# ericbrec/BSpy

Measured on AMD Instinct MI355X. Metric: M evals/sec on 10M-point bicubic (p=3x3) surface, higher is better.
Workload: dtype f64; 1 GPU; BASELINE configs[1]: bicubic surface order 4x4, nCoef 64x64, nDep 3, fp64, clamped uniform knots, Spline.evaluate on 10000000 uniform-random (u,v); points_total=10000000, points_per_gpu=10000000, op=evaluate

## Files before the change

bspy_amd/_native.py:

```python
import ctypes
import os

import numpy as np

_HERE = os.path.dirname(os.path.abspath(__file__))
LIB_PATH = os.environ.get("BSPY_AMD_LIB") or os.path.join(_HERE, "csrc", "libbspy_amd.so")

BSK_F32, BSK_F64 = 0, 1
BSK_HOST, BSK_DEVICE = 0, 1
BSK_OK, BSK_ERR_INVALID, BSK_ERR_DOMAIN, BSK_ERR_HIP, BSK_ERR_NO_DEVICE, BSK_ERR_UNSUPPORTED = range(6)
BSK_MAX_NIND, BSK_MAX_ORDER = 8, 16
BSK_INTEGRAL_MEASURE, BSK_INTEGRAL_NODES = 0, 1

PRODUCT_SYMBOLS = (
    "bsk_version", "bsk_last_error", "bsk_device_count",
    "bsk_spline_create", "bsk_spline_update", "bsk_spline_destroy",
    "bsk_evaluate", "bsk_jacobian", "bsk_normal", "bsk_curvature", "bsk_evaluate_grid", "bsk_tessellate",
    "bsk_domain_status", "bsk_bspline_values", "bsk_last_kernel",
    "bsk_multi_create", "bsk_multi_destroy", "bsk_multi_shard_plan", "bsk_multi_stream", "bsk_multi_evaluate",
    "bsk_multi_jacobian", "bsk_integral",
    "bsk_fit_create", "bsk_fit_destroy", "bsk_fit_info", "bsk_fit_solve_host", "bsk_fit_sweep", "bsk_fit_residual",
    "bsk_fit_last_kernel",
    "bsk_band_create", "bsk_band_destroy", "bsk_band_apply_host", "bsk_band_apply", "bsk_band_last_kernel",
    "bsk_band_absmax", "bsk_band_absmax_host", "bsk_band_apply_fma_host",
    "bsk_product_create", "bsk_product_destroy", "bsk_product_apply_host", "bsk_product_apply", "bsk_product_last_kernel",
    "bsk_scan_create", "bsk_scan_destroy", "bsk_scan_apply_host", "bsk_scan_apply", "bsk_scan_last_kernel",
    "bsk_sum_apply_host", "bsk_sum_apply", "bsk_sum_last_kernel",
    "bsk_roots_extract_host", "bsk_roots_flag_host", "bsk_roots_flag", "bsk_roots_isolate_host", "bsk_roots_isolate", "bsk_roots_last_kernel",
    "bsk_project_seed_host", "bsk_project_seed", "bsk_project_newton_host", "bsk_project_newton", "bsk_project_last_kernel",
    "bsk_contour_flag_host", "bsk_contour_flag", "bsk_contour_march_host", "bsk_contour_march", "bsk_contour_last_kernel",
    "bsk_iso_flag_host", "bsk_iso_flag", "bsk_iso_walk_host", "bsk_iso_walk", "bsk_iso_leaf_host", "bsk_iso_leaf", "bsk_iso_vertex_host",
    "bsk_iso_vertex", "bsk_iso_last_kernel",
    "bsk_mesh_bound_host", "bsk_mesh_bound", "bsk_mesh_count_host", "bsk_mesh_count", "bsk_mesh_emit_host", "bsk_mesh_emit",
    "bsk_mesh_vertex_host", "bsk_mesh_vertex", "bsk_mesh_last_kernel",
    "bsk_rays_boxes_host", "bsk_rays_boxes", "bsk_rays_count_host", "bsk_rays_count", "bsk_rays_emit_host", "bsk_rays_emit",
    "bsk_rays_isolate_host", "bsk_rays_isolate", "bsk_rays_reduce_host", "bsk_rays_reduce", "bsk_rays_last_kernel",
    "bsk_ssx_count_host", "bsk_ssx_count", "bsk_ssx_emit_host", "bsk_ssx_emit", "bsk_ssx_isolate_host", "bsk_ssx_isolate",
    "bsk_ssx_merge_host", "bsk_ssx_merge", "bsk_ssx_last_kernel",
    "bsk_scatter_key_host", "bsk_scatter_key", "bsk_scatter_gram_host", "bsk_scatter_gram", "bsk_scatter_cell_host", "bsk_scatter_cell",
    "bsk_scatter_fold_host", "bsk_scatter_fold", "bsk_scatter_residual_host", "bsk_scatter_residual", "bsk_scatter_solve_host",
    "bsk_scatter_solve_work", "bsk_scatter_solve", "bsk_scatter_reweight_host", "bsk_scatter_reweight", "bsk_scatter_last_kernel",
)
INTERNAL_SYMBOLS = ("bsk_debug_probe", "bsk_debug_stage_times", "bsk_debug_fill_lds", "bsk_debug_scatter_solve")
SYMBOLS = PRODUCT_SYMBOLS + INTERNAL_SYMBOLS
ROOTS2_SYMBOLS = ("bsk_roots2_flag_host", "bsk_roots2_flag", "bsk_roots2_isolate_host", "bsk_roots2_isolate", "bsk_roots2_merge_host",
                  "bsk_roots2_merge", "bsk_roots2_last_kernel")
ROOTS3_SYMBOLS = ("bsk_roots3_flag_host", "bsk_roots3_flag", "bsk_roots3_isolate_host", "bsk_roots3_isolate", "bsk_roots3_merge_host",
                  "bsk_roots3_merge", "bsk_roots3_last_kernel", "bsk_roots3_walk_bound")


class NativeLibraryError(RuntimeError):
    """libbspy_amd.so is missing or failed to load."""


class BskError(RuntimeError):

    def __init__(self, status, message):
        super().__init__(f"libbspy_amd status {status}: {message}")
        self.status = status


class DomainError(Exception):

    def __init__(self, index):
        super().__init__(f"parameter outside domain at flat index {index}")
        self.index = int(index)
# ... 199 lines not shown
    L.bsk_scatter_gram_host.argtypes = gram_s
    L.bsk_scatter_gram.argtypes = gram_s + [_vp]
    L.bsk_scatter_cell_host.argtypes = cell_s
    L.bsk_scatter_cell.argtypes = cell_s + [_vp]
    L.bsk_scatter_fold_host.argtypes = fold_s
    L.bsk_scatter_fold.argtypes = fold_s + [_vp]
    L.bsk_scatter_residual_host.argtypes = residual_s
    L.bsk_scatter_residual.argtypes = residual_s + [_vp]
    L.bsk_scatter_solve_host.argtypes = fold_s + [_i64p]
    reweight_s = [ctypes.c_int, ctypes.c_double, _vp, _vp, _vp, _i64, _vp]
    L.bsk_scatter_solve_work.argtypes = [ctypes.c_int] * 3 + [_i64, _i64, ctypes.c_int, _i64p]
    L.bsk_scatter_solve.argtypes = fold_s + [_vp, _i64, _vp, _vp]
    L.bsk_debug_scatter_solve.argtypes = fold_s + [_vp, _i64, _vp, ctypes.c_int, _vp]
    L.bsk_scatter_reweight_host.argtypes = reweight_s
    L.bsk_scatter_reweight.argtypes = reweight_s + [_vp]
    L.bsk_scatter_last_kernel.argtypes = []
    L.bsk_scatter_last_kernel.restype = ctypes.c_char_p
    L.bsk_last_kernel.argtypes = [_vp]
    L.bsk_last_kernel.restype = ctypes.c_char_p
    L.bsk_debug_probe.argtypes = [_vp, ctypes.c_int, ctypes.c_int, ctypes.c_int, _i64, _vp, _vp, _i64, _vp, _vp]
    L.bsk_debug_stage_times.argtypes = [_vp, ctypes.c_int, ctypes.POINTER(ctypes.c_float), ctypes.POINTER(ctypes.c_char_p),
                                        ctypes.c_int, _ip]
    L.bsk_debug_fill_lds.argtypes = [_vp, ctypes.c_uint32, ctypes.c_int, _i64p, _vp]
    for name in SYMBOLS + ROOTS2_SYMBOLS + ROOTS3_SYMBOLS:
        if name not in ("bsk_version", "bsk_last_error", "bsk_last_kernel", "bsk_fit_last_kernel", "bsk_band_last_kernel",
                        "bsk_product_last_kernel", "bsk_scan_last_kernel", "bsk_sum_last_kernel", "bsk_roots_last_kernel",
                        "bsk_roots2_last_kernel", "bsk_roots3_last_kernel", "bsk_project_last_kernel", "bsk_contour_last_kernel", "bsk_iso_last_kernel", "bsk_mesh_last_kernel", "bsk_rays_last_kernel",
                        "bsk_ssx_last_kernel", "bsk_scatter_last_kernel"):
            getattr(L, name).restype = ctypes.c_int
    _lib = L
    return L


def check(status, first_bad=None):
    if status == BSK_OK:
        return
    if status == BSK_ERR_DOMAIN:
        raise DomainError(first_bad.value if first_bad is not None else -1)
    raise BskError(status, lib().bsk_last_error().decode("utf-8", "replace"))


def device_count():
    n = ctypes.c_int(0)
    st = lib().bsk_device_count(ctypes.byref(n))
    if st != BSK_OK:
        return 0
# ... 17 lines not shown
```

bspy_amd/csrc/bsk_api.hip:

```cpp
#include "bsk_kernels.hpp"
#include "bsk_tile.hpp"
#include "bsk_stream.hpp"
#include "bsk_rowrot.hpp"
#include "bsk_uniform.hpp"
#include "bsk_rec32.hpp"
#include "bsk_host.hpp"

#include <condition_variable>
#include <mutex>
#include <thread>

struct HostPipe;
static void pipe_destroy(HostPipe *p);

static int ceil_log2(int x)
{
    int s = 0;
    while ((1 << s) < x) ++s;
    return s;
}

template <typename T>
static void build_axis_table(const T *knots, int order, int nk, std::vector<T> &tab)
{
// ... 21 lines not shown
static int lut_buckets(int order, int ncoef)
{
    int m = 16;
    while (m < 4 * (ncoef - order + 1) && m < 4096) m <<= 1;
    return m;
}

template <typename T>
static void build_lut(const T *knots, int order, int ncoef, int m, T &scale, int &steps, std::vector<unsigned> &lut)
{
    const double lo = (double)knots[order - 1], hi = (double)knots[ncoef];
    const double w = hi - lo;
    scale = T((double)m / w);
    const double inv = 1.0 / (double)scale;
    int widest = 0;
    for (int b = 0; b < m; ++b) {
        const int l = host_span<T>(knots, order, ncoef, lo + ((double)b - 0.01) * inv);
        const int h = (b == m - 1) ? ncoef : host_span<T>(knots, order, ncoef, lo + ((double)b + 1.01) * inv);
        widest = std::max(widest, h - l);
        lut.push_back((unsigned)l | ((unsigned)h << 16));
    }
    steps = ceil_log2(widest + 1);
}

template <typename T>
static bsk_status upload_tables(bsk_spline s, const void *const *knots, const void *coefs)
{
    Desc<T> &d = desc_of<T>(s);
    TileDesc<T> &td = tile_of<T>(s);
    std::vector<T> tab;
    std::vector<unsigned> lut;
    for (int iv = 0; iv < s->nInd; ++iv) {
        d.off[iv] = (int)tab.size();
        const T *k = static_cast<const T *>(knots[iv]);
        build_axis_table<T>(k, s->order[iv], d.nk[iv], tab);
        d.lo[iv] = k[s->order[iv] - 1];
        d.hi[iv] = k[s->ncoef[iv]];
        td.lut_off[iv] = (int)lut.size();
        const int m_alloc = lut_buckets(s->order[iv], s->ncoef[iv]);
        int m_small = 16;
        while (m_small < s->ncoef[iv] - s->order[iv] + 1) m_small <<= 1;
        std::vector<unsigned> seg;
        int m_use = m_alloc;
        if (m_small < m_alloc) {
            build_lut<T>(k, s->order[iv], s->ncoef[iv], m_small, td.lut_scale[iv], td.lut_steps[iv], seg);
            if (td.lut_steps[iv] <= 1) m_use = m_small;
// ... 2 lines not shown
            seg.clear();
            build_lut<T>(k, s->order[iv], s->ncoef[iv], m_alloc, td.lut_scale[iv], td.lut_steps[iv], seg);
        }
        td.lut_m[iv] = m_use;
        seg.resize((size_t)m_alloc, seg.empty() ? 0u : seg.back());
        lut.insert(lut.end(), seg.begin(), seg.end());
    }
    if ((int)tab.size() != d.tab_len) return fail(BSK_ERR_INVALID, "internal: axis table size changed");
    if ((int)lut.size() != td.lut_len) return fail(BSK_ERR_INVALID, "internal: bucket table size changed");
    HIPCHK(hipSetDevice(s->device));
    if (d.tab_len) HIPCHK(hipMemcpy(s->tab, tab.data(), sizeof(T) * tab.size(), hipMemcpyHostToDevice));
    s->tab_host.assign(reinterpret_cast<const unsigned char *>(tab.data()),
                       reinterpret_cast<const unsigned char *>(tab.data()) + sizeof(T) * tab.size());
    if (td.lut_len) HIPCHK(hipMemcpy(s->lut, lut.data(), sizeof(unsigned) * lut.size(), hipMemcpyHostToDevice));
    if (d.coef_len) HIPCHK(hipMemcpy(s->coef, coefs, sizeof(T) * (size_t)d.coef_len, hipMemcpyHostToDevice));
    if (s->coef_aos) {
        const size_t cells = (size_t)d.coef_len / (size_t)s->nDep;
        std::vector<T> aos((size_t)d.coef_len);
        const T *src = static_cast<const T *>(coefs);
        for (int dep = 0; dep < s->nDep; ++dep)
            for (size_t c = 0; c < cells; ++c) aos[c * s->nDep + dep] = src[(size_t)dep * cells + c];
        HIPCHK(hipMemcpy(s->coef_aos, aos.data(), sizeof(T) * aos.size(), hipMemcpyHostToDevice));
    }
    return BSK_OK;
}

template <typename T>
static bsk_status init_desc(bsk_spline s)
{
    Desc<T> &d = desc_of<T>(s);
    memset(&d, 0, sizeof(d));
    d.nInd = s->nInd;
    d.nDep = s->nDep;
    long long clen = 1;
    long long tlen = 0;
    for (int iv = 0; iv < s->nInd; ++iv) {
        d.order[iv] = s->order[iv];
        d.ncoef[iv] = s->ncoef[iv];
        d.nk[iv] = s->order[iv] + s->ncoef[iv];
        d.steps[iv] = ceil_log2(s->ncoef[iv] - s->order[iv] + 1);
        tlen += (long long)s->order[iv] * d.nk[iv];
        clen *= s->ncoef[iv];
    }
    d.cstride[s->nInd] = 1;
    for (int iv = s->nInd - 1; iv >= 0; --iv) {
        const long long st = (long long)d.cstride[iv + 1] * s->ncoef[iv];
        if (st * std::max(1, s->nDep) > 0x7fffffffLL) return fail(BSK_ERR_UNSUPPORTED, "coefficient table exceeds 2^31 elements");
// ... 105 lines not shown
    s->num_cu = prop.multiProcessorCount > 0 ? prop.multiProcessorCount : 256;
    s->lds_max = std::min<size_t>(160 * 1024, prop.maxSharedMemoryPerMultiProcessor > 0
                                                  ? (size_t)prop.maxSharedMemoryPerMultiProcessor
                                                  : (size_t)64 * 1024);
    HIPCHK_C(hipMalloc(&s->tab, std::max<size_t>(16, s->esize * (size_t)tab_len)));
    HIPCHK_C(hipMalloc(&s->coef, std::max<size_t>(16, s->esize * (size_t)coef_len)));
    {
        const size_t tbytes = s->esize * (size_t)tab_len + s->esize * (size_t)coef_len;
        const int omax = max_order(s);
        const bool fixed = nInd <= 3 && omax <= 6;
        if (fixed && nDep <= 4 && tbytes + 8192 > s->lds_max)
            HIPCHK_C(hipMalloc(&s->coef_aos, std::max<size_t>(16, s->esize * (size_t)coef_len)));
        else if (fixed && nDep <= 4 && nInd == 2 && !s->same_order && omax >= 2) {
            HIPCHK_C(hipMalloc(&s->coef_aos, std::max<size_t>(16, s->esize * (size_t)coef_len)));
            s->aos_small = true;
        }
    }
    HIPCHK_C(hipMalloc((void **)&s->lut, std::max<size_t>(16, sizeof(unsigned) * (size_t)(dtype == BSK_F32 ? s->t32.lut_len : s->t64.lut_len))));
    HIPCHK_C(hipMalloc((void **)&s->bad, 2 * sizeof(unsigned long long)));
    if (const char *v = getenv("BSK_VARIANT")) s->variant = atoi(v);
    HIPCHK_C(hipMemset(s->bad, 0xff, 2 * sizeof(unsigned long long)));
#undef HIPCHK_C
    st = upload_all(s, knots, coefs);
    if (st != BSK_OK) { s->uni_img.release(); cleanup(); return st; }
    *out = s;
    return BSK_OK;
}

extern "C" bsk_status bsk_spline_update(bsk_spline s, const void *const *knots, const void *coefs)
{
    if (!s || !knots || !coefs) return fail(BSK_ERR_INVALID, "NULL argument");
    HIPCHK(hipSetDevice(s->device));
    HIPCHK(hipDeviceSynchronize());
    return upload_all(s, knots, coefs);
}

extern "C" bsk_status bsk_spline_destroy(bsk_spline s)
{
    if (!s) return BSK_OK;
    (void)hipSetDevice(s->device);
    (void)hipDeviceSynchronize();
    if (s->tab) (void)hipFree(s->tab);
    if (s->coef) (void)hipFree(s->coef);
    if (s->bad) (void)hipFree(s->bad);
    if (s->lut) (void)hipFree(s->lut);
    if (s->coef_aos) (void)hipFree(s->coef_aos);
    s->in_ws.release();
    s->out_ws.release();
    s->aux_ws.release();
    s->curv_ws.release();
    s->bin_ws.release();
    if (s->ticket) (void)hipFree(s->ticket);
    s->ticket = nullptr;
    s->uni_img.release();
    if (s->pin) (void)hipHostFree(s->pin);
    s->pin = nullptr;
    pipe_destroy(s->pipe);
    s->pipe = nullptr;
    for (hipEvent_t &e : s->stage_ev)
        if (e) { (void)hipEventDestroy(e); e = nullptr; }
    delete s;
    return BSK_OK;
}

struct Plan {
    bool lds_coefs;
    size_t lds_bytes;
    int block, grid;
};

template <typename T>
static Plan make_plan(bsk_spline s, long long n)
{
    const Desc<T> &d = desc_of<T>(s);
    Plan p;
    const size_t tab_b = sizeof(T) * (size_t)((d.tab_len + 1) & ~1);
    const size_t coef_b = sizeof(T) * (size_t)d.coef_len;
// ... 106 lines not shown
    return rec_b + rr_lut_bytes<T>(tdr.lut_len) + coef_b + TILE * sizeof(unsigned);
}

template <typename T>
static bool rowrot_applies(bsk_spline s)
{
    return has_fixed_path(s) && s->nInd == 2 && (s->order[0] == 2 || s->order[0] == 4) &&
           (s->variant == 0 || s->variant == 9) && rowrot_lds_bytes<T>(s) <= s->lds_max;
}

static bool axis_tables_fit_lds(bsk_spline s)
{
    const size_t tab_len = s->dtype == BSK_F32 ? (size_t)s->d32.tab_len : (size_t)s->d64.tab_len;
    return s->esize * (tab_len + 2) + 1024 <= s->lds_max;
}

struct PointShape {
    int omax;
    bool fixed;
    size_t lds;
    bool axis_lds;
    size_t lds_rowrot;
    bool rowrot;
    bool uni, uniN;
    bool lds_curve;
    bool lds_nd;
};

template <typename T>
static PointShape point_shape(bsk_spline s)
{
    PointShape ps;
    ps.omax = max_order(s);
    ps.fixed = has_fixed_path(s);
    ps.lds = tile_lds_bytes<T>(s);
    ps.axis_lds = axis_tables_fit_lds(s);
    ps.rowrot = rowrot_applies<T>(s);
    ps.lds_rowrot = ps.rowrot ? rowrot_lds_bytes<T>(s) : 0;
    ps.uni = s->uni;
    ps.uniN = s->uniN;
    ps.lds_curve = s->nInd == 1 && s->order[0] >= 6 && s->order[0] <= 8 && s->variant != 1 && ps.lds != 0;
    ps.lds_nd = ps.fixed && s->variant != 1 && s->order[0] <= 5 && ps.lds != 0;
    return ps;
}

template <int LO, int HI, typename F>
static bsk_status with_nind_order(bsk_spline s, F &&f)
{
    return with_range<1, 3>(s->nInd, [&](auto ni) {
        return with_range<LO, HI>(s->order[0], [&](auto o) { return f(ni, o); });
    });
}

template <typename T>
static bool axis_is_uniform(const T *k, int order, int ncoef, bool &clamp_lo, bool &clamp_hi)
{
    const int ns = ncoef - order + 1;
    const long double lo = k[order - 1], hi = k[ncoef];
    if (!(hi > lo) || ns < 1) return false;
    const long double h = (hi - lo) / ns;
    const long double eps = std::numeric_limits<T>::epsilon();
// ... 58 lines not shown
    for (int i = 0; i < O; ++i)
        for (int j = 0; j < i; ++j) {
            if (std::fabs(C[(size_t)i * O + j]) > 1e-15L) return false;
            C[(size_t)i * O + j] = 0;
        }
    M = C;
    return true;
}

static void unclamp_axis(std::vector<long double> &w, size_t outer, int nc, size_t inner, int O,
                         const std::vector<long double> &M, bool low)
{
    std::vector<long double> p(O);
    for (size_t a = 0; a < outer; ++a)
        for (size_t c = 0; c < inner; ++c) {
            long double *line = w.data() + a * (size_t)nc * inner + c;
            for (int i = 0; i < O; ++i) p[i] = line[(size_t)(low ? i : nc - 1 - i) * inner];
            for (int i = 0; i < O; ++i) {
                long double q = 0;
                for (int j = 0; j < O; ++j) q += M[(size_t)i * O + j] * p[j];
                line[(size_t)(low ? i : nc - 1 - i) * inner] = q;
            }
        }
}

template <typename T>
static bsk_status upload_uniform(bsk_spline s, const void *const *knots, const void *coefs)
{
    s->uni = false;
    if (!rowrot_applies<T>(s) || s->variant == 9) return BSK_OK;
    bool cl[2][2];
    for (int iv = 0; iv < 2; ++iv) {
        if (s->ncoef[iv] < 2 * s->order[iv]) return BSK_OK;
        if (!axis_is_uniform<T>(static_cast<const T *>(knots[iv]), s->order[iv], s->ncoef[iv], cl[iv][0], cl[iv][1])) return BSK_OK;
    }
    const int O = s->order[0];
    if (sizeof(T) == 4 && O > 2) return BSK_OK;
    std::vector<long double> M;
    if (!unclamp_matrix(O, M)) return BSK_OK;
    const int nc0 = s->ncoef[0], nc1 = s->ncoef[1], nDep = s->nDep;
    std::vector<long double> w((size_t)nDep * nc0 * nc1);
    const T *src = static_cast<const T *>(coefs);
    for (size_t i = 0; i < w.size(); ++i) w[i] = src[i];
    if (cl[0][0]) unclamp_axis(w, (size_t)nDep, nc0, (size_t)nc1, O, M, true);
    if (cl[0][1]) unclamp_axis(w, (size_t)nDep, nc0, (size_t)nc1, O, M, false);
    if (cl[1][0]) unclamp_axis(w, (size_t)nDep * nc0, nc1, 1, O, M, true);
// ... 165 lines not shown
            if (ps.rowrot) {
                if (ps.uni) {
                    const UniDesc<T> &ud = uni_of<T>(s);
                    const size_t lds_u = (size_t)ud.img_bytes + TILE * sizeof(unsigned);
                    return with_int<1, 2, 3, 0>(s->nDep, [&](auto nd) {
                        return for_rr_chunks<T>(s, prm, n, [&](const Params<T> &cp, long long m, long long n0) {
                            return launch(s, "eval_uni", eval_uni<T, O, DERIV, decltype(nd)::value>, rr_grid(s, m, lds_u),
                                          dim3(TILE), lds_u, st, ud, s->uni_img.p, cp, (unsigned)m, n0, out + n0, ostride, w,
                                          s->bad);
                        });
                    });
                }
                if constexpr (sizeof(T) == 4 && O == 4) {
                    const size_t lds_r = r32_lds_bytes(s->ncoef[0] - 3, s->ncoef[1] - 3, td.lut_len, s->ncoef[0], s->ncoef[1]);
                    if (s->variant == 0 && s->nDep >= 1 && s->nDep <= 4 && lds_r + 256 <= s->lds_max)
                        return with_int<1, 2, 3, 4>(s->nDep, [&](auto nd) {
                            return for_rr_chunks<T>(s, prm, n, [&](const Params<T> &cp, long long m, long long n0) {
                                return launch(s, "eval_rec32", eval_rec32<DERIV, decltype(nd)::value>, rr_grid(s, m, lds_r),
                                              dim3(TILE), lds_r, st, d, td, tab, s->lut, coef, cp, (unsigned)m, n0, out + n0,
                                              ostride, w, s->bad);
                            });
                        });
                }
                const size_t lds_rr = ps.lds_rowrot;
                return with_int<1, 2, 3, 0>(s->nDep, [&](auto nd) {
                    return for_rr_chunks<T>(s, prm, n, [&](const Params<T> &cp, long long m, long long n0) {
                        return launch(s, "eval_rowrot", eval_rowrot<T, O, DERIV, decltype(nd)::value>, rr_grid(s, m, lds_rr),
                                      dim3(TILE), lds_rr, st, d, td, tab, s->lut, coef, cp, (unsigned)m, n0, out + n0, ostride,
                                      w, s->bad);
                    });
                });
            }
        }
        if constexpr (O <= 5) {
            if (ps.uniN) {
                const UniDescN<T> &un = uniN_of<T>(s);
                const size_t lds_u = un.img_bytes;
                return launch(s, "eval_stream_uni", eval_stream_uni<T, NIND, O, DERIV>,
                              dim3(persistent_grid(s, ntiles, lds_per_cu(s, lds_u))), dim3(STREAM_BLOCK), lds_u, st, d, un,
                              s->uni_img.p, prm, n, out, ostride, w, s->bad);
            }
        }
        return launch(s, "eval_stream", eval_stream<T, NIND, O, DERIV>, dim3(persistent_grid(s, ntiles, lds_per_cu(s, lds))),
                      dim3(STREAM_BLOCK), lds, st, d, td, tab, s->lut, coef, prm, n, out, ostride, w, s->bad);
    });
}
// ... 971 lines not shown
                                         const void *u, int64_t n, int derivative_order, int taylor_coefs,
                                         const int32_t *knot_in, int32_t *ix_out, void *basis_out)
{
    if (!knots || !u || !ix_out || !basis_out) return fail(BSK_ERR_INVALID, "NULL argument");
    if (order < 1 || order > MAXO) return fail(BSK_ERR_UNSUPPORTED, "order must be in [1, BSK_MAX_ORDER]");
    if (nknots < 2 * order) return fail(BSK_ERR_INVALID, "need at least 2 * order knots");
    if (derivative_order < 0) return fail(BSK_ERR_INVALID, "negative derivative order");
    if (n < 0) return fail(BSK_ERR_INVALID, "negative count");
    if (n == 0) return BSK_OK;
    if (knot_in)
        for (int64_t i = 0; i < n; ++i)
            if (knot_in[i] < order || knot_in[i] > nknots - order)
                return fail(BSK_ERR_INVALID, "explicit knot index outside [order, len(knots) - order]");
    if (dtype != BSK_F32 && dtype != BSK_F64) return fail(BSK_ERR_INVALID, "dtype must be BSK_F32 or BSK_F64");
    return with_dtype(dtype, [&](auto z) {
        using T = decltype(z);
        return run_basis<T>(device, static_cast<const T *>(knots), nknots, order, static_cast<const T *>(u), n,
                            derivative_order, taylor_coefs, knot_in, ix_out, static_cast<T *>(basis_out));
    });
}

extern "C" const char *bsk_last_kernel(bsk_spline s) { return s ? s->last_kernel : ""; }

extern "C" bsk_status bsk_debug_stage_times(bsk_spline s, int enable, float *ms, const char **names, int cap, int *count)
{
    if (!s) return fail(BSK_ERR_INVALID, "spline is NULL");
    int n = 0;
    if (ms && names && count && s->stage_count > 1) {
        HIPCHK(hipSetDevice(s->device));
        HIPCHK(hipEventSynchronize(s->stage_ev[s->stage_count - 1]));
        for (int i = 0; i + 1 < s->stage_count && n < cap; ++i, ++n) {
            HIPCHK(hipEventElapsedTime(&ms[n], s->stage_ev[i], s->stage_ev[i + 1]));
            names[n] = s->stage_name[i + 1];
        }
    }
    if (count) *count = n;
    s->stage_timing = enable != 0;
    if (!enable) s->stage_count = 0;
    return BSK_OK;
}

extern "C" bsk_status bsk_debug_probe(bsk_spline s, int mode, int blocks_per_cu, int threads, int64_t lds_bytes,
                                      const void *u, const void *v, int64_t n, void *out, void *stream)
{
    if (!s || !u || !v || !out) return fail(BSK_ERR_INVALID, "NULL argument");
    HIPCHK(hipSetDevice(s->device));
// ... 42 lines not shown
```

bspy_amd/csrc/bsk_host.hpp:

```cpp
#pragma once
#include <algorithm>
#include <cmath>
#include <cstdio>
#include <cstring>
#include <limits>
#include <string>
#include <tuple>
#include <type_traits>
#include <utility>
#include <vector>

#include "bsk_common.hpp"
#include "bsk_tile.hpp"

using namespace bsk;

inline thread_local std::string g_err;

inline bsk_status fail(bsk_status st, const std::string &msg)
{
    g_err = msg;
    return st;
}

#define HIPCHK(expr)                                                                          \
    do {                                                                                      \
        hipError_t e_ = (expr);                                                               \
        if (e_ != hipSuccess)                                                                 \
            return fail(BSK_ERR_HIP, std::string(#expr) + ": " + hipGetErrorString(e_));      \
    } while (0)

struct DevBuf {
    void *p = nullptr;
    size_t cap = 0;
    hipError_t reserve(size_t bytes)
    {
// ... 29 lines not shown
    void *coef = nullptr;
    void *coef_aos = nullptr;
    unsigned *lut = nullptr;
    int variant = 0;
    unsigned long long *bad = nullptr;
    int num_cu = 256;
    size_t lds_max = 160 * 1024;
    DevBuf in_ws, out_ws, aux_ws;
    DevBuf bin_ws;
    unsigned *ticket = nullptr;
    bool bin_reuse = false;
    DevBuf curv_ws;
    std::vector<unsigned char> tab_host;
    void *pin = nullptr;
    size_t pin_cap = 0;
    struct HostPipe *pipe = nullptr;
    bool uni = false;
    UniDesc<float> u32;
    UniDesc<double> u64;
    DevBuf uni_img;
    bool uniN = false;
    UniDescN<float> un32;
    UniDescN<double> un64;
    const char *last_kernel = "";
    static constexpr int MAX_STAGES = 12;
    bool stage_timing = false;
    hipEvent_t stage_ev[MAX_STAGES] = {};
    const char *stage_name[MAX_STAGES] = {};
    int stage_count = 0;
};

inline void stage_mark(bsk_spline s, hipStream_t st, const char *name, bool first = false)
{
    if (!s->stage_timing) return;
    if (first) s->stage_count = 0;
    if (s->stage_count >= bsk_spline_s::MAX_STAGES) return;
    hipEvent_t &e = s->stage_ev[s->stage_count];
    if (!e && hipEventCreateWithFlags(&e, hipEventDefault) != hipSuccess) { e = nullptr; return; }
    if (hipEventRecord(e, st) != hipSuccess) return;
    s->stage_name[s->stage_count++] = name;
}

template <typename T>
Desc<T> &desc_of(bsk_spline s);
template <>
inline Desc<float> &desc_of<float>(bsk_spline s) { return s->d32; }
template <>
// ... 34 lines not shown
}

inline int max_order(bsk_spline s)
{
    return *std::max_element(s->order, s->order + s->nInd);
}

inline int persistent_grid(bsk_spline s, long long units, long long per_cu)
{
    return (int)std::max<long long>(1, std::min<long long>(units, (long long)s->num_cu * per_cu));
}

inline int lds_per_cu(bsk_spline s, size_t lds_bytes)
{
    return (int)std::max<size_t>(1, std::min<size_t>(2, s->lds_max / lds_bytes));
}

template <typename K, typename... Args>
inline bsk_status launch(bsk_spline s, const char *name, K kernel, dim3 grid, dim3 block, size_t lds, hipStream_t st,
                         const Args &...args)
{
    HIPCHK(allow_lds(kernel, lds));
    if (name) s->last_kernel = name;
    hipLaunchKernelGGL(kernel, grid, block, lds, st, args...);
    HIPCHK(hipGetLastError());
    return BSK_OK;
}

template <int BLOCK, typename K, typename... Args>
inline bsk_status launch_lanes(K kernel, long long lanes, long long layers, hipStream_t st, const Args &...args)
{
    hipLaunchKernelGGL(kernel, dim3((unsigned)((lanes + BLOCK - 1) / BLOCK), (unsigned)layers), dim3(BLOCK), 0, st, args...);
    HIPCHK(hipGetLastError());
    return BSK_OK;
}
template <int BLOCK, typename K, typename... Args>
inline bsk_status launch_lanes(K kernel, long long lanes, hipStream_t st, const Args &...args)
{
    return launch_lanes<BLOCK>(kernel, lanes, 1, st, args...);
}

template <int N>
using int_c = std::integral_constant<int, N>;
template <typename F>
inline bsk_status with_bool(bool b, F &&f)
{
// ... 36 lines not shown
```

bspy_amd/csrc/bsk_rowrot.hpp:

```cpp
#pragma once
#include "bsk_stream.hpp"

namespace bsk {

constexpr unsigned RR_MAX_CHUNK = 1u << 28;

template <typename T, int O>
__host__ __device__ constexpr unsigned rr_rec_bytes() { return (unsigned)((O | 1) * sizeof(T)); }

template <typename T, int O>
__host__ __device__ inline unsigned rr_records_bytes(int nk0, int nk1)
{
    return ((unsigned)(nk0 + nk1) * rr_rec_bytes<T, O>() + 15u) & ~15u;
}

template <typename T>
__host__ __device__ inline unsigned rr_lut_bytes(int lut_len)
{
    return ((unsigned)lut_len * (unsigned)sizeof(unsigned) + 15u) & ~15u;
}

template <typename T, int O>
__device__ __forceinline__ void stage_image_rowrot(char *smem, const Desc<T> &d, const TileDesc<T> &td,
                                                   const T *__restrict__ gtab, const unsigned *__restrict__ glut,
                                                   const T *__restrict__ gcoef, int nc1, int rs)
{
    constexpr int REC = O | 1;
    const unsigned rec_bytes = rr_records_bytes<T, O>(d.nk[0], d.nk[1]);
    T *srec = reinterpret_cast<T *>(smem);
    unsigned *slut = reinterpret_cast<unsigned *>(smem + rec_bytes);
    T *scoef = reinterpret_cast<T *>(smem + rec_bytes + rr_lut_bytes<T>(td.lut_len));
    constexpr int U = 8;
    const int bd = blockDim.x;
    for (int i0 = threadIdx.x; i0 < d.coef_len; i0 += bd * U) {
        T v[U];
#pragma unroll
        for (int k = 0; k < U; ++k) { const int i = i0 + k * bd; v[k] = i < d.coef_len ? gcoef[i] : T(0); }
#pragma unroll
        for (int k = 0; k < U; ++k) {
            const int i = i0 + k * bd;
            if (i < d.coef_len) { const int row = i / nc1, col = i - row * nc1; scoef[row * rs + col] = v[k]; }
        }
    }
// ... 479 lines not shown
```

bspy_amd/csrc/bsk_uniform.hpp:

```cpp
#pragma once
#include "bsk_rowrot.hpp"
#include "bsk_rank.hpp"

namespace bsk {

__device__ __forceinline__ void stage_linear(char *smem, const void *__restrict__ gimg, unsigned bytes)
{
    const uint4 *__restrict__ g = static_cast<const uint4 *>(gimg);
    uint4 *s = reinterpret_cast<uint4 *>(smem);
    const unsigned n16 = bytes >> 4;
    constexpr int U = 8;
    const unsigned bd = blockDim.x;
    for (unsigned i0 = threadIdx.x; i0 < n16; i0 += bd * U) {
        uint4 v[U];
#pragma unroll
        for (int k = 0; k < U; ++k) v[k] = g[min(i0 + k * bd, n16 - 1u)];
#pragma unroll
        for (int k = 0; k < U; ++k) { const unsigned i = i0 + k * bd; if (i < n16) s[i] = v[k]; }
    }
}

template <typename T, bool NANFIX>
__device__ __forceinline__ void uni_spans2(const unsigned (&kn_a)[2], const UniDesc<T> &ud, const T (&u)[2], int (&m)[2],
                                           T (&z)[2])
// ... 124 lines not shown
        b[2] = (z * T(0.5)) * z;
        b[1] = (T(1) - z) * z + T(0.5);
    } else if constexpr (O == 4) {
        const T sixth = T(1.0 / 6.0);
        const T w = T(1) - z;
        const T z2 = z * z, w2 = w * w;
        const T z3 = z2 * z;
        b[0] = (w2 * sixth) * w;
        b[3] = z3 * sixth;
        b[1] = z3 * T(0.5) + (T(2.0 / 3.0) - z2);
        b[2] = z3 * T(-0.5) + (z2 * T(0.5) + (z * T(0.5) + sixth));
    } else {
        const T c = T(1.0 / 24.0);
        const T w = T(1) - z;
        const T w2 = w * w, z2 = z * z;
        b[0] = (w2 * c) * w2;
        b[4] = (z2 * c) * z2;
        b[1] = (((T(-4.0 / 24.0) * z + T(12.0 / 24.0)) * z + T(-6.0 / 24.0)) * z + T(-12.0 / 24.0)) * z + T(11.0 / 24.0);
        b[2] = (((T(6.0 / 24.0) * z + T(-12.0 / 24.0)) * z + T(-6.0 / 24.0)) * z + T(12.0 / 24.0)) * z + T(11.0 / 24.0);
        b[3] = (((T(-4.0 / 24.0) * z + T(4.0 / 24.0)) * z + T(6.0 / 24.0)) * z + T(4.0 / 24.0)) * z + c;
    }
}

__host__ __device__ inline int uni_row_stride(int nc1, int nDep, int O)
{
    int r = nc1 * (nDep <= 3 ? nDep : 1);
    while ((r & 31) != 32 / O) ++r;
    return r;
}

template <int O>
__device__ __forceinline__ int uni_rank_ballot(int base, int lane)
{
    static_assert(O == 2 || O == 4, "32 / O classes: 4 or 3 ballots");
    return ballot_rank<(O == 4 ? 3 : 4)>((unsigned)base & (unsigned)(32 / O - 1), lane);
}
template <int O>
__device__ __forceinline__ int uni_rank_atomic(int base, unsigned *s_rc, int lane)
{
    return (int)atomicAdd(&s_rc[(lane & 32) + (base & (32 / O - 1))], 1u);
}
template <typename T, int O>
__device__ __forceinline__ int uni_rows(unsigned coef_a, int base, int rank, unsigned rstride, unsigned (&ra)[O])
{
    const int rho = (rank - (int)((unsigned)base / (unsigned)(32 / O))) & (O - 1);
    const unsigned a0 = coef_a + (unsigned)base * (unsigned)sizeof(T);
#pragma unroll
    for (int a = 0; a < O; ++a) ra[a] = a0 + __umul24((unsigned)((a + rho) & (O - 1)), rstride);
    return rho;
}

template <typename T, int O, bool DERIV, int ND>
// ... 59 lines not shown
                uni_issue_window<T, O, ND>(ra, dep, c);
            } else {
#pragma unroll
                for (int a = 0; a < O; ++a) lds_issue_row<T, O>(ra[a], c[a]);
            }
            block_wait<0>(c);
            T q[O];
#pragma unroll
            for (int a = 0; a < O; ++a) {
                T t = T(0);
#pragma unroll
                for (int k = 0; k < O; ++k) t += c[a][k] * b[1][k];
                q[a] = mul_rn<T>(t, b0r[a]);
            }
            T r;
            if constexpr (O == 2) r = add_rn<T>(q[0], q[1]);
            else r = add_rn<T>(add_rn<T>(q[0], q[2]), add_rn<T>(q[1], q[3]));
            rr_store(o, off, r);
            o += ostride;
            if constexpr (ND == 0) {
#pragma unroll
                for (int a = 0; a < O; ++a) ra[a] += dstride;
            }
        }
        __builtin_amdgcn_s_setprio(0);
    }
}

template <typename T, int O, bool NORMAL, int ND>
__global__ __launch_bounds__(TILE) void jac_uni(const UniDesc<T> ud, const void *__restrict__ gimg, const Params<T> prm,
                                                const unsigned N, const long long n0, T *__restrict__ out,
                                                const long long ostride, unsigned long long *bad, const int normalize,
                                                const int negate)
{
    static_assert(O == 2 || O == 4, "row rotation covers orders 2 and 4");
    static_assert(!NORMAL || ND == 3, "the fused normal is a surface in 3-D");
    constexpr int CS = ND > 0 ? ND : 1;
    extern __shared__ __attribute__((aligned(16))) char smem[];
    const unsigned kn_a[2] = {(unsigned)(size_t)smem + ud.kn_off[0], (unsigned)(size_t)smem + ud.kn_off[1]};
    const unsigned coef_a = (unsigned)(size_t)smem + ud.coef_off;
    const int rs = ud.rs;
    const unsigned rstride = (unsigned)rs * (unsigned)sizeof(T);
    const unsigned dstride = (unsigned)(ud.ncoef[0] * rs) * (unsigned)sizeof(T);
    const int lane = threadIdx.x & 63;
    const unsigned stride = gridDim.x * (unsigned)TILE;
    unsigned n = ((threadIdx.x >> 6) * gridDim.x + blockIdx.x) * 64u + (unsigned)lane;
// ... 310 lines not shown
```

include/bspy_amd.h:

```cpp
#ifndef BSPY_AMD_H
#define BSPY_AMD_H

#include <stdint.h>

#ifdef __cplusplus
extern "C" {
#endif

#define BSK_VERSION 1

#define BSK_MAX_NIND 8
#define BSK_MAX_ORDER 16

typedef enum { BSK_F32 = 0, BSK_F64 = 1 } bsk_dtype;
typedef enum { BSK_HOST = 0, BSK_DEVICE = 1 } bsk_mem;

typedef enum {
    BSK_OK = 0,
    BSK_ERR_INVALID = 1,
    BSK_ERR_DOMAIN = 2,
    BSK_ERR_HIP = 3,
    BSK_ERR_NO_DEVICE = 4,
    BSK_ERR_UNSUPPORTED = 5
} bsk_status;
// ... 376 lines not shown
bsk_status bsk_bspline_values(bsk_dtype dtype, int device, const void *knots, int nknots, int order,
                              const void *u, int64_t n, int derivative_order, int taylor_coefs,
                              const int32_t *knot_in, int32_t *ix_out, void *basis_out);

typedef struct bsk_multi_s *bsk_multi;
bsk_status bsk_multi_create(bsk_dtype dtype, int ndev, const int *devices , int nInd, int nDep,
                            const int *order, const int *nCoef, const void *const *knots, const void *coefs,
                            bsk_multi *out);
bsk_status bsk_multi_destroy(bsk_multi m);
bsk_status bsk_multi_shard_plan(bsk_multi m, int64_t n, int64_t *start );
bsk_status bsk_multi_stream(bsk_multi m, int d, void **stream );
bsk_status bsk_multi_evaluate(bsk_multi m, const int *wrt, const void *const *uvw, int64_t n, bsk_mem mem,
                              void *const *out, int gather, int64_t *first_bad);
bsk_status bsk_multi_jacobian(bsk_multi m, const void *const *uvw, int64_t n, bsk_mem mem, void *const *out,
                              int gather, int64_t *first_bad);

const char *bsk_last_kernel(bsk_spline s);

#ifdef BSK_INTERNAL
bsk_status bsk_debug_probe(bsk_spline s, int mode, int blocks_per_cu, int threads, int64_t lds_bytes,
                           const void *u, const void *v, int64_t n, void *out, void *stream);
bsk_status bsk_debug_stage_times(bsk_spline s, int enable, float *ms, const char **names, int cap, int *count);
bsk_status bsk_debug_fill_lds(bsk_spline s, uint32_t pattern, int mode, int64_t *mismatches, void *stream);
bsk_status bsk_debug_scatter_solve(int nind, int K0, int K1, int64_t n0, int64_t n1, int ndep, const double *stencil,
                                   const double *rhs, double *coefs, double *work, int64_t work_doubles, int64_t *bad_row,
                                   int stages, void *stream);
#endif

#ifdef __cplusplus
}
#endif
#endif
```

Before: 114,200 M evals/s.

## Prebuild row-rotation LDS image on host and stage it linearly in eval kernel

Adds a host-built, control-point-major image (knot records, span LUT, padded coefficient rows) that is uploaded once at spline creation. A new eval_rowrot_img kernel copies this image into LDS with a single linear stage instead of rebuilding the layout per block, then runs the same row-rotation evaluation. The aim is to cut per-block staging and transpose work in the prologue. It costs extra device memory and a second code path that is used only for large point counts and nDep up to 3. A debug query for last-launch geometry is also added.

```diff
diff --git a/bspy_amd/_native.py b/bspy_amd/_native.py
--- a/bspy_amd/_native.py
+++ b/bspy_amd/_native.py
@@ -41,7 +41,8 @@
     "bsk_scatter_fold_host", "bsk_scatter_fold", "bsk_scatter_residual_host", "bsk_scatter_residual", "bsk_scatter_solve_host",
     "bsk_scatter_solve_work", "bsk_scatter_solve", "bsk_scatter_reweight_host", "bsk_scatter_reweight", "bsk_scatter_last_kernel",
 )
-INTERNAL_SYMBOLS = ("bsk_debug_probe", "bsk_debug_stage_times", "bsk_debug_fill_lds", "bsk_debug_scatter_solve")
+INTERNAL_SYMBOLS = ("bsk_debug_probe", "bsk_debug_stage_times", "bsk_debug_fill_lds", "bsk_debug_last_launch",
+                    "bsk_debug_scatter_solve")
 SYMBOLS = PRODUCT_SYMBOLS + INTERNAL_SYMBOLS
 ROOTS2_SYMBOLS = ("bsk_roots2_flag_host", "bsk_roots2_flag", "bsk_roots2_isolate_host", "bsk_roots2_isolate", "bsk_roots2_merge_host",
                   "bsk_roots2_merge", "bsk_roots2_last_kernel")
@@ -287,6 +288,7 @@
     L.bsk_debug_stage_times.argtypes = [_vp, ctypes.c_int, ctypes.POINTER(ctypes.c_float), ctypes.POINTER(ctypes.c_char_p),
                                         ctypes.c_int, _ip]
     L.bsk_debug_fill_lds.argtypes = [_vp, ctypes.c_uint32, ctypes.c_int, _i64p, _vp]
+    L.bsk_debug_last_launch.argtypes = [_vp, _ip, _ip, _i64p]
     for name in SYMBOLS + ROOTS2_SYMBOLS + ROOTS3_SYMBOLS:
         if name not in ("bsk_version", "bsk_last_error", "bsk_last_kernel", "bsk_fit_last_kernel", "bsk_band_last_kernel",
                         "bsk_product_last_kernel", "bsk_scan_last_kernel", "bsk_sum_last_kernel", "bsk_roots_last_kernel",
diff --git a/bspy_amd/csrc/bsk_api.hip b/bspy_amd/csrc/bsk_api.hip
--- a/bspy_amd/csrc/bsk_api.hip
+++ b/bspy_amd/csrc/bsk_api.hip
@@ -67,6 +67,9 @@
     }
     steps = ceil_log2(widest + 1);
 }
+
+template <typename T>
+static bsk_status upload_rowrot_image(bsk_spline s, const T *tab, const unsigned *lut, const T *coefs);
 
 template <typename T>
 static bsk_status upload_tables(bsk_spline s, const void *const *knots, const void *coefs)
@@ -115,7 +118,7 @@
             for (size_t c = 0; c < cells; ++c) aos[c * s->nDep + dep] = src[(size_t)dep * cells + c];
         HIPCHK(hipMemcpy(s->coef_aos, aos.data(), sizeof(T) * aos.size(), hipMemcpyHostToDevice));
     }
-    return BSK_OK;
+    return upload_rowrot_image<T>(s, tab.data(), lut.data(), static_cast<const T *>(coefs));
 }
 
 template <typename T>
@@ -267,7 +270,7 @@
     HIPCHK_C(hipMemset(s->bad, 0xff, 2 * sizeof(unsigned long long)));
 #undef HIPCHK_C
     st = upload_all(s, knots, coefs);
-    if (st != BSK_OK) { s->uni_img.release(); cleanup(); return st; }
+    if (st != BSK_OK) { s->uni_img.release(); s->rr_img.release(); cleanup(); return st; }
     *out = s;
     return BSK_OK;
 }
@@ -298,6 +301,7 @@
     if (s->ticket) (void)hipFree(s->ticket);
     s->ticket = nullptr;
     s->uni_img.release();
+    s->rr_img.release();
     if (s->pin) (void)hipHostFree(s->pin);
     s->pin = nullptr;
     pipe_destroy(s->pipe);
@@ -450,6 +454,7 @@
     bool axis_lds;
     size_t lds_rowrot;
     bool rowrot;
+    bool rr_img;
     bool uni, uniN;
     bool lds_curve;
     bool lds_nd;
@@ -465,6 +470,7 @@
     ps.axis_lds = axis_tables_fit_lds(s);
     ps.rowrot = rowrot_applies<T>(s);
     ps.lds_rowrot = ps.rowrot ? rowrot_lds_bytes<T>(s) : 0;
+    ps.rr_img = ps.rowrot && s->rr_img_ok;
     ps.uni = s->uni;
     ps.uniN = s->uniN;
     ps.lds_curve = s->nInd == 1 && s->order[0] >= 6 && s->order[0] <= 8 && s->variant != 1 && ps.lds != 0;
@@ -569,6 +575,27 @@
                 line[(size_t)(low ? i : nc - 1 - i) * inner] = q;
             }
         }
+}
+
+template <typename T>
+static bsk_status upload_rowrot_image(bsk_spline s, const T *tab, const unsigned *lut, const T *coefs)
+{
+    s->rr_img_ok = false;
+    if (!rowrot_applies<T>(s) || s->nDep > 3) return BSK_OK;
+    const Desc<T> &d = desc_of<T>(s);
+    const TileDesc<T> &td = tile_of<T>(s);
+    bool fits = false;
+    const RrImage lay = rr_image_layout<T>(s->order[0], s->ncoef[0], s->ncoef[1], s->nDep, td.lut_len, s->lds_max, fits);
+    if (!fits) return BSK_OK;
+    std::vector<unsigned char> img(lay.bytes);
+    const T *const axis[2] = {tab + d.off[0], tab + d.off[1]};
+    rr_image_fill<T>(lay, s->order[0], s->ncoef[0], s->ncoef[1], s->nDep, axis, lut, td.lut_len, coefs, img.data());
+    HIPCHK(hipSetDevice(s->device));
+    HIPCHK(s->rr_img.reserve(lay.bytes));
+    HIPCHK(hipMemcpy(s->rr_img.p, img.data(), lay.bytes, hipMemcpyHostToDevice));
+    s->rr_lay = lay;
+    s->rr_img_ok = true;
+    return BSK_OK;
 }
 
 template <typename T>
@@ -780,6 +807,17 @@
                             });
                         });
                 }
+                if (ps.rr_img && n >= RR_IMG_MIN_POINTS) {
+                    const RrImage &lay = s->rr_lay;
+                    const size_t lds_i = lay.bytes;
+                    return with_int<1, 2, 3>(s->nDep, [&](auto nd) {
+                        return for_rr_chunks<T>(s, prm, n, [&](const Params<T> &cp, long long m, long long n0) {
+                            return launch(s, "eval_rowrot", eval_rowrot_img<T, O, DERIV, decltype(nd)::value>,
+                                          rr_grid(s, m, lds_i), dim3(TILE), lds_i, st, d, td, (const void *)s->rr_img.p,
+                                          lay.bytes, lay.rs, cp, (unsigned)m, n0, out + n0, ostride, w, s->bad);
+                        });
+                    });
+                }
                 const size_t lds_rr = ps.lds_rowrot;
                 return with_int<1, 2, 3, 0>(s->nDep, [&](auto nd) {
                     return for_rr_chunks<T>(s, prm, n, [&](const Params<T> &cp, long long m, long long n0) {
@@ -1797,6 +1835,15 @@
 
 extern "C" const char *bsk_last_kernel(bsk_spline s) { return s ? s->last_kernel : ""; }
 
+extern "C" bsk_status bsk_debug_last_launch(bsk_spline s, int *grid, int *block, int64_t *lds_bytes)
+{
+    if (!s) return fail(BSK_ERR_INVALID, "NULL handle");
+    if (grid) *grid = s->last_grid;
+    if (block) *block = s->last_block;
+    if (lds_bytes) *lds_bytes = (int64_t)s->last_lds;
+    return BSK_OK;
+}
+
 extern "C" bsk_status bsk_debug_stage_times(bsk_spline s, int enable, float *ms, const char **names, int cap, int *count)
 {
     if (!s) return fail(BSK_ERR_INVALID, "spline is NULL");
diff --git a/bspy_amd/csrc/bsk_host.hpp b/bspy_amd/csrc/bsk_host.hpp
--- a/bspy_amd/csrc/bsk_host.hpp
+++ b/bspy_amd/csrc/bsk_host.hpp
@@ -12,6 +12,7 @@
 
 #include "bsk_common.hpp"
 #include "bsk_tile.hpp"
+#include "bsk_rr_image.hpp"
 
 using namespace bsk;
 
@@ -87,7 +88,12 @@
     bool uniN = false;
     UniDescN<float> un32;
     UniDescN<double> un64;
+    bool rr_img_ok = false;
+    RrImage rr_lay = {};
+    DevBuf rr_img;
     const char *last_kernel = "";
+    int last_grid = 0, last_block = 0;
+    size_t last_lds = 0;
     static constexpr int MAX_STAGES = 12;
     bool stage_timing = false;
     hipEvent_t stage_ev[MAX_STAGES] = {};
@@ -168,6 +174,9 @@
 {
     HIPCHK(allow_lds(kernel, lds));
     if (name) s->last_kernel = name;
+    s->last_grid = (int)grid.x;
+    s->last_block = (int)block.x;
+    s->last_lds = lds;
     hipLaunchKernelGGL(kernel, grid, block, lds, st, args...);
     HIPCHK(hipGetLastError());
     return BSK_OK;
diff --git a/bspy_amd/csrc/bsk_rowrot.hpp b/bspy_amd/csrc/bsk_rowrot.hpp
--- a/bspy_amd/csrc/bsk_rowrot.hpp
+++ b/bspy_amd/csrc/bsk_rowrot.hpp
@@ -1,24 +1,11 @@
 #pragma once
 #include "bsk_stream.hpp"
+#include "bsk_rr_image.hpp"
 
 namespace bsk {
 
 constexpr unsigned RR_MAX_CHUNK = 1u << 28;
 
-template <typename T, int O>
-__host__ __device__ constexpr unsigned rr_rec_bytes() { return (unsigned)((O | 1) * sizeof(T)); }
-
-template <typename T, int O>
-__host__ __device__ inline unsigned rr_records_bytes(int nk0, int nk1)
-{
-    return ((unsigned)(nk0 + nk1) * rr_rec_bytes<T, O>() + 15u) & ~15u;
-}
-
-template <typename T>
-__host__ __device__ inline unsigned rr_lut_bytes(int lut_len)
-{
-    return ((unsigned)lut_len * (unsigned)sizeof(unsigned) + 15u) & ~15u;
-}
 
 template <typename T, int O>
 __device__ __forceinline__ void stage_image_rowrot(char *smem, const Desc<T> &d, const TileDesc<T> &td,
diff --git a/bspy_amd/csrc/bsk_rr_image.hpp b/bspy_amd/csrc/bsk_rr_image.hpp
--- /dev/null
+++ b/bspy_amd/csrc/bsk_rr_image.hpp
@@ -0,0 +1,83 @@
+#pragma once
+#include <cstddef>
+#include <cstring>
+
+#if defined(__HIPCC__) || defined(__CUDACC__)
+#define BSK_IMG_HD __host__ __device__
+#else
+#define BSK_IMG_HD
+#endif
+
+namespace bsk {
+
+template <typename T, int O>
+BSK_IMG_HD constexpr unsigned rr_rec_bytes() { return (unsigned)((O | 1) * sizeof(T)); }
+
+template <typename T, int O>
+BSK_IMG_HD inline unsigned rr_records_bytes(int nk0, int nk1)
+{
+    return ((unsigned)(nk0 + nk1) * rr_rec_bytes<T, O>() + 15u) & ~15u;
+}
+
+template <typename T>
+BSK_IMG_HD inline unsigned rr_lut_bytes(int lut_len)
+{
+    return ((unsigned)lut_len * (unsigned)sizeof(unsigned) + 15u) & ~15u;
+}
+
+BSK_IMG_HD inline int uni_row_stride(int nc1, int nDep, int O)
+{
+    int r = nc1 * (nDep <= 3 ? nDep : 1);
+    while ((r & 31) != 32 / O) ++r;
+    return r;
+}
+
+struct RrImage {
+    unsigned rec_off[2];
+    unsigned lut_off;
+    unsigned coef_off;
+    unsigned bytes;
+    int rs;
+};
+
+template <typename T>
+inline RrImage rr_image_layout(int O, int nc0, int nc1, int nDep, int lut_len, size_t limit, bool &fits)
+{
+    RrImage L;
+    const int nk0 = O + nc0, nk1 = O + nc1;
+    const size_t rec_stride = (size_t)(O | 1) * sizeof(T);
+    const size_t rec_b = ((size_t)(nk0 + nk1) * rec_stride + 15) & ~(size_t)15;
+    const size_t lut_b = ((size_t)lut_len * sizeof(unsigned) + 15) & ~(size_t)15;
+    L.rs = uni_row_stride(nc1, nDep, O);
+    const size_t coef_b = ((size_t)nc0 * (size_t)L.rs * sizeof(T) + 15) & ~(size_t)15;
+    const size_t total = rec_b + lut_b + coef_b;
+    fits = total <= limit && total < ((size_t)1 << 31);
+    L.rec_off[0] = 0;
+    L.rec_off[1] = (unsigned)((size_t)nk0 * rec_stride);
+    L.lut_off = (unsigned)rec_b;
+    L.coef_off = (unsigned)(rec_b + lut_b);
+    L.bytes = fits ? (unsigned)total : 0u;
+    return L;
+}
+
+template <typename T>
+inline void rr_image_fill(const RrImage &L, int O, int nc0, int nc1, int nDep, const T *const (&tab)[2],
+                          const unsigned *lut, int lut_len, const T *coefs, unsigned char *img)
+{
+    memset(img, 0, L.bytes);
+    const int rec = O | 1;
+    const int nk[2] = {O + nc0, O + nc1};
+    for (int iv = 0; iv < 2; ++iv) {
+        T *r = reinterpret_cast<T *>(img + L.rec_off[iv]);
+        for (int D = 0; D < O; ++D)
+            for (int k = 0; k < nk[iv]; ++k) r[(size_t)k * rec + D] = tab[iv][(size_t)D * nk[iv] + k];
+    }
+    if (lut_len) memcpy(img + L.lut_off, lut, (size_t)lut_len * sizeof(unsigned));
+    T *c = reinterpret_cast<T *>(img + L.coef_off);
+    for (int dep = 0; dep < nDep; ++dep)
+        for (int i0 = 0; i0 < nc0; ++i0)
+            for (int i1 = 0; i1 < nc1; ++i1)
+                c[(size_t)i0 * L.rs + (size_t)i1 * nDep + dep] = coefs[((size_t)dep * nc0 + i0) * nc1 + i1];
+}
+
+}
diff --git a/bspy_amd/csrc/bsk_uniform.hpp b/bspy_amd/csrc/bsk_uniform.hpp
--- a/bspy_amd/csrc/bsk_uniform.hpp
+++ b/bspy_amd/csrc/bsk_uniform.hpp
@@ -170,12 +170,6 @@
     }
 }
 
-__host__ __device__ inline int uni_row_stride(int nc1, int nDep, int O)
-{
-    int r = nc1 * (nDep <= 3 ? nDep : 1);
-    while ((r & 31) != 32 / O) ++r;
-    return r;
-}
 
 template <int O>
 __device__ __forceinline__ int uni_rank_ballot(int base, int lane)
@@ -281,6 +275,84 @@
 #pragma unroll
                 for (int a = 0; a < O; ++a) ra[a] += dstride;
             }
+        }
+        __builtin_amdgcn_s_setprio(0);
+    }
+}
+
+constexpr long long RR_IMG_MIN_POINTS = 1ll << 18;
+
+template <typename T, int O, bool DERIV, int ND>
+__global__ __launch_bounds__(TILE) void eval_rowrot_img(const Desc<T> d, const TileDesc<T> td, const void *__restrict__ gimg,
+                                                        const unsigned img_bytes, const int rs, const Params<T> prm,
+                                                        const unsigned N, const long long n0, T *__restrict__ out,
+                                                        const long long ostride, const Wrt wrt, unsigned long long *bad)
+{
+    static_assert(O == 2 || O == 4, "row rotation covers orders 2 and 4");
+    static_assert(ND >= 1 && ND <= 3, "control-point-major image: nDep is a template constant");
+    extern __shared__ __attribute__((aligned(16))) char smem[];
+    const unsigned rec_a[2] = {(unsigned)(size_t)smem, (unsigned)(size_t)smem + (unsigned)d.nk[0] * rr_rec_bytes<T, O>()};
+    const unsigned lut_a = rec_a[0] + rr_records_bytes<T, O>(d.nk[0], d.nk[1]);
+    const unsigned coef_a = lut_a + rr_lut_bytes<T>(td.lut_len);
+    const unsigned rstride = (unsigned)rs * (unsigned)sizeof(T);
+    const int lane = threadIdx.x & 63;
+    const int steps = td.lut_steps[0] > td.lut_steps[1] ? td.lut_steps[0] : td.lut_steps[1];
+    const unsigned stride = gridDim.x * (unsigned)TILE;
+    unsigned n = ((threadIdx.x >> 6) * gridDim.x + blockIdx.x) * 64u + (unsigned)lane;
+    const T lo0 = d.lo[0], lo1 = d.lo[1], hi0 = d.hi[0], hi1 = d.hi[1];
+    const T *p0 = prm.p[0], *p1 = prm.p[1];
+    T un[2] = {lo0, lo1};
+    if (n < N) { un[0] = rr_load(p0, n * (unsigned)sizeof(T)); un[1] = rr_load(p1, n * (unsigned)sizeof(T)); }
+    stage_linear(smem, gimg, img_bytes);
+    __syncthreads();
+    asm volatile("" : "+v"(un[0]), "+v"(un[1]));
+
+    for (; n < N; n += stride) {
+        const T u[2] = {un[0], un[1]};
+        const bool outside = (u[0] < lo0) | (u[0] > hi0) | (u[1] < lo1) | (u[1] > hi1);
+        {
+            const unsigned nn = min(n + stride, N - 1u) * (unsigned)sizeof(T);
+            un[0] = rr_load(p0, nn);
+            un[1] = rr_load(p1, nn);
+        }
+        if (outside) record_bad(bad, n0 + (long long)n);
+
+        int ix[2];
+        rr_find_spans<T, O, DERIV>(rec_a, lut_a, d, td, steps, u, ix);
+        const int base = (int)__umul24((unsigned)(ix[0] - O), (unsigned)rs) + (ix[1] - O) * ND;
+        const int rank = uni_rank_ballot<O>(base, lane);
+        T b[2][O];
+        {
+            T kn[2][O], rc[2][O][O];
+            rr_issue_tables<T, O>(rec_a, ix, kn, rc);
+            bases_compute<T, 2, O, DERIV, 0>(u, wrt, kn, rc, b);
+        }
+        unsigned ra[O];
+        const int rho = uni_rows<T, O>(coef_a, base, rank, rstride, ra);
+        T b0r[O];
+        rotate_basis_values<T, O>(b[0], rho, b0r);
+
+        const unsigned off = n * (unsigned)sizeof(T);
+        T *o = out;
+        __builtin_amdgcn_s_setprio(3);
+#pragma unroll
+        for (int dep = 0; dep < ND; ++dep) {
+            T c[O][O];
+            uni_issue_window<T, O, ND>(ra, dep, c);
+            block_wait<0>(c);
+            T q[O];
+#pragma unroll
+            for (int a = 0; a < O; ++a) {
+                T t = T(0);
+#pragma unroll
+                for (int k = 0; k < O; ++k) t += c[a][k] * b[1][k];
+                q[a] = mul_rn<T>(t, b0r[a]);
+            }
+            T r;
+            if constexpr (O == 2) r = add_rn<T>(q[0], q[1]);
+            else r = add_rn<T>(add_rn<T>(q[0], q[2]), add_rn<T>(q[1], q[3]));
+            rr_store(o, off, r);
+            o += ostride;
         }
         __builtin_amdgcn_s_setprio(0);
     }
diff --git a/include/bspy_amd.h b/include/bspy_amd.h
--- a/include/bspy_amd.h
+++ b/include/bspy_amd.h
@@ -422,6 +422,7 @@
                            const void *u, const void *v, int64_t n, void *out, void *stream);
 bsk_status bsk_debug_stage_times(bsk_spline s, int enable, float *ms, const char **names, int cap, int *count);
 bsk_status bsk_debug_fill_lds(bsk_spline s, uint32_t pattern, int mode, int64_t *mismatches, void *stream);
+bsk_status bsk_debug_last_launch(bsk_spline s, int *grid, int *block, int64_t *lds_bytes);
 bsk_status bsk_debug_scatter_solve(int nind, int K0, int K1, int64_t n0, int64_t n1, int ndep, const double *stencil,
                                    const double *rhs, double *coefs, double *work, int64_t work_doubles, int64_t *bad_row,
                                    int stages, void *stream);
```

New measurement: 114,400 M evals/s, median of 3. Within noise of the previous version (+0.2%).
